# LabJunBMI/E3-invaraint-diffusion-model

Measured on AMD Instinct MI355X. Metric: denoising-steps/sec (batched pocket graphs), higher is better.
Workload: dtype f32 storage and accumulation, f16x3 products (fp32 grade); 1 GPU; structure_model sampling step, 256 x 256-residue pockets per GPU, 12+12 layers x 768, T=1000 schedule, encoder recomputed every step (as the reference); pockets_per_gpu=256, seq_len=256, parallelism=pocket-sharded x1, no collective

## Files before the change

e3-invaraint-diffusion-model_amd/csrc/attn_relkey_coop.hip:

```cpp
#include <type_traits>

#include "e3d_common.h"

namespace {

typedef __bf16 bf16x8 __attribute__((ext_vector_type(8)));
typedef __bf16 bf16x4 __attribute__((ext_vector_type(4)));
typedef _Float16 f16x8 __attribute__((ext_vector_type(8)));
typedef _Float16 f16x4 __attribute__((ext_vector_type(4)));
template <typename E> struct AV;
template <> struct AV<__bf16> { typedef bf16x8 x8; typedef bf16x4 x4; };
template <> struct AV<_Float16> { typedef f16x8 x8; typedef f16x4 x4; };
template <typename X> struct Elem;
template <> struct Elem<bf16x8> { typedef __bf16 type; };
template <> struct Elem<bf16x4> { typedef __bf16 type; };
template <> struct Elem<f16x8> { typedef _Float16 type; };
template <> struct Elem<f16x4> { typedef _Float16 type; };
__device__ __forceinline__ f32x16 mma16(const bf16x8 a, const bf16x8 b, const f32x16 c) {
    return __builtin_amdgcn_mfma_f32_32x32x16_bf16(a, b, c, 0, 0, 0);
}
__device__ __forceinline__ f32x16 mma16(const f16x8 a, const f16x8 b, const f32x16 c) {
    return __builtin_amdgcn_mfma_f32_32x32x16_f16(a, b, c, 0, 0, 0);
}

// ... 78 lines not shown
    const float* src = e + row * D + 16 * kb + 8 * (lane >> 5);
    typename AV<E>::x8 out;
    unsigned amax = 0;
#pragma unroll
    for (int t = 0; t < 8; ++t) {
        const float v = src[t];
        const E hi = (E)v;
        out[t] = plane ? (E)(v - (float)hi) : hi;
        e3d_absmax_accum(amax, v);
    }
    frag[i] = out;
    if (e_absmax && plane == 0) e3d_absmax_commit(amax, e_absmax, lane);
}

#ifdef E3D_ATTN_STAMPS
__device__ long long e3d_attn_stamps[16][8];
#define ASTAMP(slot)                                                                                     \
    do {                                                                                                 \
        if (blockIdx.x == 1000 && wid == 1 && lane == 0 && kt < 16) e3d_attn_stamps[kt][slot] = __builtin_readcyclecounter(); \
    } while (0)
#define KSTAMP(i)                                                                                        \
    do {                                                                                                 \
        if (blockIdx.x == 1000 && wid == 1 && lane == 0) e3d_attn_stamps[15][i] = __builtin_readcyclecounter(); \
    } while (0)
#else
#define ASTAMP(slot) do {} while (0)
#define KSTAMP(i) do {} while (0)
#endif

template <int W, bool RELKEY, typename E, bool DROP = false>
__global__ __launch_bounds__(W * 64, 2) void attn_coop_kernel(
    const float* __restrict__ q, int64_t q_bs, int64_t q_rs, const float* __restrict__ k, int64_t k_bs,
    int64_t k_rs, const float* __restrict__ v, int64_t v_bs, int64_t v_rs, const typename AV<E>::x8* __restrict__ e_frag,
    int P, const float* __restrict__ key_mask, float* __restrict__ out, float* __restrict__ lse, int nh, int Lq, int Lk,
    int groups_per_bh, int skip_padded_tiles, E3dBounds bnd, float rescale_tau, E3dDrop drop_in) {
    const E3dDrop drop = e3d_drop_resolve(drop_in);
    typedef typename AV<E>::x8 bf16x8;
    typedef typename AV<E>::x4 bf16x4;
    extern __shared__ __attribute__((aligned(16))) unsigned char smem_raw[];
    constexpr int NT = W * 64, NI = 512 / NT;
    const int tid = threadIdx.x, lane = tid & 63, wid = tid >> 6;
    const int qi = lane & 31, half = lane >> 5;
    const int blk = xcd_remap(blockIdx.x, gridDim.x);
    const int grp = blk % groups_per_bh, bh = blk / groups_per_bh, h = bh % nh, b = bh / nh;
    const int q0 = (grp * W + wid) * 32;
    float* ring = reinterpret_cast<float*>(smem_raw + 2 * KV_BUF_B) + wid * RING_F;
    KSTAMP(0);

    const float* kb_ = k + b * k_bs + h * D;
    const float* vb_ = v + b * v_bs + h * D;
    const float* mb = key_mask ? key_mask + (int64_t)b * Lk : nullptr;
    f32x4 qraw[8];
    {
        const float* qrow = q + b * q_bs + (int64_t)min(q0 + qi, Lq - 1) * q_rs + h * D + 8 * half;
#pragma unroll
        for (int kb = 0; kb < 4; ++kb) {
            qraw[2 * kb] = *reinterpret_cast<const f32x4*>(qrow + 16 * kb);
            qraw[2 * kb + 1] = *reinterpret_cast<const f32x4*>(qrow + 16 * kb + 4);
        }
    }
    uint64_t drop_row = 0;
    if (DROP) drop_row = e3d_drop_attn_row(drop, b, h, nh, Lq, Lk, min(q0 + qi, Lq - 1));
    const bool scan_mask = mb && skip_padded_tiles && e3d_mask_skip_is_exact(bnd);
    float mv[4];
    {
        const float* mp = mb ? mb : kb_;
#pragma unroll
        for (int c = 0; c < 4; ++c) mv[c] = mp[min(64 * c + lane, Lk - 1)];
    }

    bf16x8 qf[4][2];
    int k_tiles = (Lk + 31) >> 5;

    constexpr bool DEEP = NI <= 2;
    constexpr int NSET = DEEP ? 2 : 1;
    f32x4 sk[NSET][NI], sv[NSET][NI];
    float smask[NSET];
    int voff_k[NI], voff_v[NI];
#pragma unroll
    for (int i = 0; i < NI; ++i) {
        const int f = tid + NT * i;
        voff_k[i] = ((f >> 4) * (int)k_rs + 4 * (f & 15)) * 4;
        voff_v[i] = ((f >> 4) * (int)v_rs + 4 * (f & 15)) * 4;
    }
    const int voff_m = (tid & 31) * 4;
    auto tile_rsrc = [&](const float* base, int64_t rs, int r0, int tail_floats) {
        const int rows = Lk - r0;
        return __builtin_amdgcn_make_buffer_rsrc(const_cast<float*>(base + (int64_t)r0 * rs), 0,
                                                 (int)(((int64_t)(rows - 1) * rs + tail_floats) * 4), 0x00020000);
    };
    auto stage_load = [&](auto set_tag, int r0) {
        constexpr int SET = decltype(set_tag)::value;
        const auto rk = tile_rsrc(kb_, k_rs, r0, D), rv = tile_rsrc(vb_, v_rs, r0, D);
#pragma unroll
        for (int i = 0; i < NI; ++i) {
            sk[SET][i] = __builtin_bit_cast(f32x4, __builtin_amdgcn_raw_buffer_load_b128(rk, voff_k[i], 0, 0));
            sv[SET][i] = __builtin_bit_cast(f32x4, __builtin_amdgcn_raw_buffer_load_b128(rv, voff_v[i], 0, 0));
        }
        const auto rm = tile_rsrc(mb ? mb : kb_, 1, r0, 1);
        const float mval = __builtin_bit_cast(float, __builtin_amdgcn_raw_buffer_load_b32(rm, voff_m, 0, 0));
        smask[SET] = mb ? mval : 1.0f;
    };
    auto stage_store = [&](auto set_tag, int r0, unsigned char* buf) {
        constexpr int SET = decltype(set_tag)::value;
#pragma unroll
        for (int i = 0; i < NI; ++i) {
            const int f = tid + NT * i, row = f >> 4, c4 = f & 15;
            bf16x4 hi, lo;
            split4x2(sk[SET][i], hi, lo);
            *reinterpret_cast<bf16x4*>(buf + row * K_ROW_B + 8 * c4) = hi;
            *reinterpret_cast<bf16x4*>(buf + K_PLANE_B + row * K_ROW_B + 8 * c4) = lo;
            split4x2(sv[SET][i], hi, lo);
            *reinterpret_cast<bf16x4*>(buf + 2 * K_PLANE_B + row * V_ROW_B + 8 * c4) = hi;
            *reinterpret_cast<bf16x4*>(buf + 2 * K_PLANE_B + V_PLANE_B + row * V_ROW_B + 8 * c4) = lo;
        }
        if (tid < 32)
            reinterpret_cast<float*>(buf + 2 * K_PLANE_B + 2 * V_PLANE_B)[tid] =
                r0 + tid < Lk ? (1.0f - smask[SET]) * MASK_BIAS : -INFINITY;
    };
    using Set0 = std::integral_constant<int, 0>;
    using Set1 = std::integral_constant<int, DEEP ? 1 : 0>;

    bf16x8 ef[4][2];
    const int J0 = (Lk + 31) >> 5, qt = q0 >> 5;
    const auto e_rsrc = __builtin_amdgcn_make_buffer_rsrc(const_cast<bf16x8*>(e_frag ? e_frag : reinterpret_cast<const bf16x8*>(k)), 0,
                                                          2 * ((Lk + 31) >> 5) * 512 * 16, 0x00020000);
    const int voff_e = lane * 16;
    auto e_load = [&](int j) {
        const int so = __builtin_amdgcn_readfirstlane(j * 8192);
#pragma unroll
        for (int kb = 0; kb < 4; ++kb) {
            ef[kb][0] = __builtin_bit_cast(bf16x8, __builtin_amdgcn_raw_buffer_load_b128(e_rsrc, voff_e + kb * 1024, so, 0));
            ef[kb][1] = __builtin_bit_cast(bf16x8, __builtin_amdgcn_raw_buffer_load_b128(e_rsrc, voff_e + kb * 1024, so + 4096, 0));
        }
    };
    auto dot_q_acc = [&](const bf16x8 (&x)[4][2], f32x16 acc) {
#pragma unroll
        for (int kb = 0; kb < 4; ++kb) acc = mfma3(x[kb], qf[kb], acc);
        return acc;
    };
    auto dot_q = [&](const bf16x8 (&x)[4][2]) {
        f32x16 acc;
#pragma unroll
        for (int r = 0; r < 16; ++r) acc[r] = 0.f;
        return dot_q_acc(x, acc);
    };

    stage_load(Set0{}, 0);
    if (RELKEY) e_load(qt + J0);

    if (scan_mask) {
        int last = -1;
#pragma unroll
        for (int c = 0; c < 4; ++c) {
            const bool valid = 64 * c + lane < Lk && mv[c] != 0.f;
            const unsigned long long bits = __ballot(valid);
            if (bits) last = 64 * c + 63 - __builtin_clzll(bits);
        }
        for (int base = 256; base < Lk; base += 64) {
            const int key = base + lane;
            const bool valid = key < Lk && mb[key] != 0.f;
            const unsigned long long bits = __ballot(valid);
            if (bits) last = base + 63 - __builtin_clzll(bits);
        }
        if (last >= 0) k_tiles = (last >> 5) + 1;
    }
#pragma unroll
    for (int kb = 0; kb < 4; ++kb) {
        const f32x4 lo4 = qraw[2 * kb], hi4 = qraw[2 * kb + 1];
        float x[8] = {lo4[0] * Q_SCALE, lo4[1] * Q_SCALE, lo4[2] * Q_SCALE, lo4[3] * Q_SCALE,
                      hi4[0] * Q_SCALE, hi4[1] * Q_SCALE, hi4[2] * Q_SCALE, hi4[3] * Q_SCALE};
#pragma unroll
        for (int j = 0; j < 8; ++j) asm volatile("" : "+v"(x[j]));
        split8x2(x, qf[kb][0], qf[kb][1]);
    }
    if (RELKEY) {
        f32x16 t = dot_q(ef);
        e_load(qt - 1 + J0);
#pragma unroll
        for (int r = 0; r < 16; ++r) ring[(32 + mfma32_row(r, half)) * RING_LD + qi] = t[r];
        t = dot_q(ef);
        e_load(qt - (k_tiles > 1 ? 1 : 0) - 1 + J0);
#pragma unroll
        for (int r = 0; r < 16; ++r) ring[mfma32_row(r, half) * RING_LD + qi] = t[r];
    }
    stage_store(Set0{}, 0, smem_raw);
    if (DEEP) stage_load(Set1{}, (k_tiles > 1 ? 1 : 0) * 32);
    __syncthreads();
    KSTAMP(1);

    f32x16 o0, o1;
#pragma unroll
    for (int r = 0; r < 16; ++r) { o0[r] = 0.f; o1[r] = 0.f; }
    float m_run = 0.f, l_run = 0.f;
    float* const ring_w = ring + 4 * half * RING_LD + qi;
    const float* const ring_e = ring + (qi + 31 - 4 * half - 27) * RING_LD + qi;
    int rd_odd[16];
    if (RELKEY) {
#pragma unroll
        for (int r = 0; r < 16; ++r) rd_odd[r] = (((qi - mfma32_row(r, half) + 31) ^ 32) * RING_LD + qi);
    }

    auto tile = [&](auto par_tag, int kt) {
        constexpr int PAR = decltype(par_tag)::value;
        const unsigned char* buf = smem_raw + PAR * KV_BUF_B;
        const bool more = kt + 1 < k_tiles;
        const int kt_next = more ? kt + 1 : kt;
        ASTAMP(0);
        ASTAMP(1);

        const float* kbias = reinterpret_cast<const float*>(buf + 2 * K_PLANE_B + 2 * V_PLANE_B);
        f32x16 s;
#pragma unroll
        for (int g = 0; g < 4; ++g) {
            const f32x4 bv = *reinterpret_cast<const f32x4*>(kbias + 8 * g + 4 * half);
#pragma unroll
            for (int j = 0; j < 4; ++j) s[4 * g + j] = bv[j] - m_run;
        }
        if (RELKEY) {
#pragma unroll
            for (int r = 0; r < 16; ++r)
                s[r] += PAR ? ring[rd_odd[r]] : ring_e[(27 - ((r & 3) + 8 * (r >> 2))) * RING_LD];
        }
        {
            bf16x8 kf[4][2];
            const unsigned char* kr = buf + qi * K_ROW_B + 16 * half;
#pragma unroll
            for (int kb = 0; kb < 4; ++kb) {
                kf[kb][0] = *reinterpret_cast<const bf16x8*>(kr + 32 * kb);
                kf[kb][1] = *reinterpret_cast<const bf16x8*>(kr + K_PLANE_B + 32 * kb);
            }
            s = dot_q_acc(kf, s);
        }
        ASTAMP(2);
        const int kt_ld = DEEP ? (kt + 2 < k_tiles ? kt + 2 : k_tiles - 1) : kt_next;
        if (PAR == 0) stage_load(Set0{}, kt_ld * 32);
        else stage_load(Set1{}, kt_ld * 32);
        ASTAMP(3);

        float tmax = -INFINITY;
#pragma unroll
        for (int r = 0; r < 16; ++r) tmax = fmaxf(tmax, s[r]);
        tmax = fmaxf(tmax, __shfl_xor(tmax, 32, 64));
        const bool grow = kt == 0 || tmax > rescale_tau;
        if (__builtin_amdgcn_ballot_w64(grow) != 0ull) {
            const float delta = grow ? tmax : 0.f;
            const float alpha = kt == 0 ? 0.f : __builtin_amdgcn_exp2f(-delta);
            m_run += delta;
            l_run *= alpha;
#pragma unroll
            for (int r = 0; r < 16; ++r) { o0[r] *= alpha; o1[r] *= alpha; s[r] -= delta; }
        }
        float psum = 0.f;
#pragma unroll
        for (int r = 0; r < 16; ++r) {
            s[r] = __builtin_amdgcn_exp2f(s[r]);
            psum += s[r];
        }
        l_run += psum;
        if (DROP) {
#pragma unroll
            for (int g = 0; g < 4; ++g) {
                float m[4];
                e3d_drop_mult4_row(drop, drop_row, (uint32_t)(kt * 8 + 2 * g + half), m);
#pragma unroll
                for (int j = 0; j < 4; ++j) s[4 * g + j] *= m[j];
            }
        }
        ASTAMP(4);

        const unsigned char* vr = buf + 2 * K_PLANE_B + (4 * half + ((lane >> 2) & 3)) * V_ROW_B +
                                  2 * (16 * ((lane >> 4) & 1) + 4 * (lane & 3));
#pragma unroll
        for (int st = 0; st < 2; ++st) {
            float pv[8];
#pragma unroll
            for (int j = 0; j < 8; ++j) pv[j] = s[8 * st + j];
            bf16x8 pb[2], a0[2], a1[2];
            split8x2(pv, pb[0], pb[1]);
            const unsigned char* v0 = vr + 16 * st * V_ROW_B;
#pragma unroll
            for (int pl = 0; pl < 2; ++pl) {
                a0[pl] = tr_read8<bf16x8>(v0 + pl * V_PLANE_B, v0 + pl * V_PLANE_B + 8 * V_ROW_B);
                a1[pl] = tr_read8<bf16x8>(v0 + pl * V_PLANE_B + 64, v0 + pl * V_PLANE_B + 8 * V_ROW_B + 64);
            }
            o0 = mfma3(a0, pb, o0);
            o1 = mfma3(a1, pb, o1);
        }

        ASTAMP(5);
        if (more) {
            if (DEEP == (PAR == 0)) stage_store(Set1{}, kt_next * 32, smem_raw + (PAR ^ 1) * KV_BUF_B);
            else stage_store(Set0{}, kt_next * 32, smem_raw + (PAR ^ 1) * KV_BUF_B);
        }
        ASTAMP(6);
        if (RELKEY && more) {
            const f32x16 t = dot_q(ef);
            e_load(qt - (kt + 2 < k_tiles ? kt + 2 : k_tiles - 1) - 1 + J0);
#pragma unroll
            for (int r = 0; r < 16; ++r) ring_w[(32 * (PAR ^ 1) + (r & 3) + 8 * (r >> 2)) * RING_LD] = t[r];
        }
        __syncthreads();
        ASTAMP(7);
    };
    for (int kt = 0; kt < k_tiles; kt += 2) {
        tile(std::integral_constant<int, 0>{}, kt);
        if (kt + 1 < k_tiles) tile(std::integral_constant<int, 1>{}, kt + 1);
    }

    KSTAMP(2);
    const float l_tot = l_run + __shfl_xor(l_run, 32, 64);
    const float inv = 1.0f / l_tot;
    __builtin_amdgcn_wave_barrier();
#pragma unroll
    for (int g = 0; g < 4; ++g) {
        f32x4 a, c;
#pragma unroll
        for (int j = 0; j < 4; ++j) { a[j] = o0[4 * g + j] * inv; c[j] = o1[4 * g + j] * inv; }
        *reinterpret_cast<f32x4*>(ring + qi * OUT_LD + 8 * g + 4 * half) = a;
        *reinterpret_cast<f32x4*>(ring + qi * OUT_LD + 32 + 8 * g + 4 * half) = c;
    }
    __builtin_amdgcn_fence(__ATOMIC_RELEASE, "wavefront");
    __builtin_amdgcn_wave_barrier();
    __builtin_amdgcn_fence(__ATOMIC_ACQUIRE, "wavefront");
    float* obase = out + ((int64_t)b * Lq + q0) * (nh * D) + h * D;
#pragma unroll
    for (int i = 0; i < 8; ++i) {
        const int row = 4 * i + (lane >> 4);
        if (q0 + row < Lq)
            *reinterpret_cast<f32x4*>(obase + (int64_t)row * (nh * D) + 4 * (lane & 15)) =
                *reinterpret_cast<const f32x4*>(ring + row * OUT_LD + 4 * (lane & 15));
    }
    if (lse && half == 0 && q0 + qi < Lq) lse[((int64_t)b * nh + h) * Lq + q0 + qi] = m_run * LN2 + logf(l_tot);
    KSTAMP(3);
#ifdef E3D_ATTN_STAMPS
    asm volatile("s_waitcnt vmcnt(0)" ::: "memory");
    KSTAMP(4);
#endif
}

template <int W, bool RELKEY, typename E>
int launch_w(const float* q, int64_t q_bs, int64_t q_rs, const float* k, int64_t k_bs, int64_t k_rs, const float* v,
             int64_t v_bs, int64_t v_rs, const void* e_frag, int P, const float* key_mask,
             float* out, float* lse, int B, int nh, int Lq, int Lk, int q_tiles, int skip, E3dBounds bnd, E3dDrop drop,
             bool dropping, hipStream_t s) {
    const size_t lds = 2 * KV_BUF_B + (size_t)W * RING_F * sizeof(float);
    const int groups = q_tiles / W;
    if constexpr (std::is_same<E, __bf16>::value) {
        if (dropping) {
            static std::atomic<uint64_t> lds_ok_d{0};
            e3d_allow_lds(lds_ok_d, attn_coop_kernel<W, RELKEY, E, true>, lds);
            hipLaunchKernelGGL((attn_coop_kernel<W, RELKEY, E, true>), dim3(B * nh * groups), dim3(W * 64), lds, s, q, q_bs, q_rs,
                               k, k_bs, k_rs, v, v_bs, v_rs, reinterpret_cast<const typename AV<E>::x8*>(e_frag), P, key_mask,
                               out, lse, nh, Lq, Lk, groups, skip, bnd, g_rescale_tau, drop);
            return e3d_launch_status("e3d_relkey_attn_fwd_split (cooperative, dropout)");
        }
    }
    static std::atomic<uint64_t> lds_ok{0};
    e3d_allow_lds(lds_ok, attn_coop_kernel<W, RELKEY, E>, lds);
    hipLaunchKernelGGL((attn_coop_kernel<W, RELKEY, E>), dim3(B * nh * groups), dim3(W * 64), lds, s, q, q_bs, q_rs, k, k_bs,
                       k_rs, v, v_bs, v_rs, reinterpret_cast<const typename AV<E>::x8*>(e_frag), P, key_mask, out, lse, nh, Lq, Lk, groups, skip, bnd, g_rescale_tau, drop);
    return e3d_launch_status("e3d_relkey_attn_fwd_split (cooperative)");
}

template <bool RELKEY, typename E>
int launch_any(int W, const float* q, int64_t q_bs, int64_t q_rs, const float* k, int64_t k_bs, int64_t k_rs,
               const float* v, int64_t v_bs, int64_t v_rs, const void* e_frag, int P,
               const float* key_mask, float* out, float* lse, int B, int nh, int Lq, int Lk, int q_tiles, int skip,
               E3dBounds bnd, E3dDrop drop, bool dropping, hipStream_t s) {
#define E3D_COOP_CASE(w)                                                                                          \
    case w:                                                                                                       \
        return launch_w<w, RELKEY, E>(q, q_bs, q_rs, k, k_bs, k_rs, v, v_bs, v_rs, e_frag, P, key_mask, out, lse, B, nh, \
                                   Lq, Lk, q_tiles, skip, bnd, drop, dropping, s)
    switch (W) {
        E3D_COOP_CASE(8);
        E3D_COOP_CASE(4);
// ... 30 lines not shown
    return launch_any<true, E>(W, q, q_bs, q_rs, k, k_bs, k_rs, v, v_bs, v_rs, e_scratch, P, key_mask, out, lse, B, nh, Lq,
                               Lk, q_tiles, skip, bnd, drop, dropping, s);
}

int e3d_attn_coop_launch(const float* q, int64_t q_bs, int64_t q_rs, const float* k, int64_t k_bs, int64_t k_rs,
                         const float* v, int64_t v_bs, int64_t v_rs, const float* dist_emb, int P,
                         const float* key_mask, float* out, float* lse, int B, int nh, int Lq, int Lk, int skip,
                         E3dBounds bnd, void* e_scratch, int e_ready, int f16, E3dDrop drop, bool dropping, hipStream_t s) {
    if (f16)
        return coop_launch_t<_Float16>(q, q_bs, q_rs, k, k_bs, k_rs, v, v_bs, v_rs, dist_emb, P, key_mask, out, lse, B, nh, Lq,
                                       Lk, skip, bnd, e_scratch, e_ready, drop, dropping, s);
    return coop_launch_t<__bf16>(q, q_bs, q_rs, k, k_bs, k_rs, v, v_bs, v_rs, dist_emb, P, key_mask, out, lse, B, nh, Lq, Lk,
                                 skip, bnd, e_scratch, e_ready, drop, dropping, s);
}

extern "C" float e3d_attn_rescale_tau(float tau) {
    const float prev = g_rescale_tau;
    if (tau >= 0.f) g_rescale_tau = tau;
    return prev;
}

#ifdef E3D_ATTN_STAMPS
extern "C" int e3d_debug_read_attn_stamps(long long* host_out) {
    return (int)hipMemcpyFromSymbol(host_out, HIP_SYMBOL(e3d_attn_stamps), sizeof(long long) * 16 * 8);
}
#endif

int e3d_attn_fill_planes(const float* dist_emb, int P, int Lk, void* scratch, int f16, float* e_absmax, hipStream_t s) {
    const int J0 = (Lk + 31) / 32, n_items = 2 * J0 * 512;
    if (f16)
// ... 10 lines not shown
```

e3-invaraint-diffusion-model_amd/csrc/attn_relkey_split.hip:

```cpp
#include "attn_split_frag.h"

namespace {

template <int NS, bool RELKEY, bool DROP, typename E>
__global__ __launch_bounds__(256, 2) void attn_fwd_split_kernel(
    const float* __restrict__ q, int64_t q_bs, int64_t q_rs, const float* __restrict__ k, int64_t k_bs,
    int64_t k_rs, const float* __restrict__ v, int64_t v_bs, int64_t v_rs, const float* __restrict__ dist_emb,
    int P, const float* __restrict__ key_mask, float* __restrict__ out, float* __restrict__ lse, int nh, int Lq,
    int Lk, int q_tiles, int n_units, int skip_padded_tiles, E3dBounds bnd, E3dDrop drop_in) {
    const E3dDrop drop = e3d_drop_resolve(drop_in);
    typedef typename AV<E>::x8 bf16x8;
    extern __shared__ __attribute__((aligned(16))) float smem[];
    const int lane = threadIdx.x & 63, wid = threadIdx.x >> 6;
    const int qi = lane & 31, half = lane >> 5;
    const int unit = xcd_remap(blockIdx.x, gridDim.x) * (blockDim.x >> 6) + wid;
    if (unit >= n_units) return;
    const int qt = unit % q_tiles, bh = unit / q_tiles, h = bh % nh, b = bh / nh;
    float* ring = smem + wid * WAVE_LDS_F;
    float* stg = ring + RING_F;
    float* kbias = stg + STG_F;

    const int q0 = qt * 32;
    const int lq = min(q0 + qi, Lq - 1);
    uint64_t drop_row = 0;
// ... 190 lines not shown
    }
    E3D_REQUIRE((int64_t)B * nh * ((Lq + 31) / 32) < (1ll << 30), "attn_split: too many tiles");
    hipStream_t s = (hipStream_t)stream;
    if (dist_emb && e_scratch && !e_scratch_ready) {
        const int rc = e3d_attn_fill_planes(dist_emb, P, Lk, e_scratch, f16, e_absmax, s);
        if (rc) return rc;
        e_scratch_ready = 1;
    }
    static int coop = -1;
    if (coop < 0) {
        const char* e = getenv("E3D_ATTN_COOP");
        coop = e ? atoi(e) : 1;
    }
    const bool dropping = drop_p > 0.f;
    const bool span_ok = (int64_t)Lk * (k_rs > v_rs ? k_rs : v_rs) * 4 < ((int64_t)1 << 31) && k_rs > 0 && v_rs > 0 &&
                         k_rs < ((int64_t)1 << 24) && v_rs < ((int64_t)1 << 24);
    if ((terms == 3 || (f16 && !dropping)) && coop && span_ok && v_rs % 4 == 0 && v_bs % 4 == 0 && ((Lq + 31) / 32) % 4 == 0 &&
        (!dist_emb || e_scratch))
        return e3d_attn_coop_launch(q, q_bs, q_rs, k, k_bs, k_rs, v, v_bs, v_rs, dist_emb, P, key_mask, out, lse, B, nh,
                                    Lq, Lk, g_skip_padded, bnd, e_scratch, e_scratch_ready, f16, d, dropping, s);
    if (dropping) {
        if (terms == 3)
            return launch<2, true>(q, q_bs, q_rs, k, k_bs, k_rs, v, v_bs, v_rs, dist_emb, P, key_mask, out, lse, B, nh, Lq, Lk, bnd, s, d);
        return launch<3, true>(q, q_bs, q_rs, k, k_bs, k_rs, v, v_bs, v_rs, dist_emb, P, key_mask, out, lse, B, nh, Lq, Lk, bnd, s, d);
    }
    if (f16)
        return launch<2, false, _Float16>(q, q_bs, q_rs, k, k_bs, k_rs, v, v_bs, v_rs, dist_emb, P, key_mask, out, lse, B, nh,
                                          Lq, Lk, bnd, s);
    if (terms == 3)
        return launch<2>(q, q_bs, q_rs, k, k_bs, k_rs, v, v_bs, v_rs, dist_emb, P, key_mask, out, lse, B, nh, Lq, Lk, bnd, s);
    return launch<3>(q, q_bs, q_rs, k, k_bs, k_rs, v, v_bs, v_rs, dist_emb, P, key_mask, out, lse, B, nh, Lq, Lk, bnd, s);
// ... 53 lines not shown
```

e3-invaraint-diffusion-model_amd/hip.py:

```python
import ctypes
import os
from ctypes import c_char_p, c_float, c_int, c_int64, c_uint32, c_uint64, c_void_p

_HERE = os.path.dirname(os.path.abspath(__file__))
LIB_PATH = os.environ.get("E3D_HIP_LIB", os.path.join(_HERE, "libe3d_hip.so"))
ABI_VERSION = 5

_P = c_void_p
_SIGNATURES = {
    "e3d_abi_version": (c_int, []),
    "e3d_last_error": (c_char_p, []),
    "e3d_gemm_bias_act_f32": (c_int, [_P, c_int64, _P, _P, _P, c_int64, c_int, c_int, c_int, c_int, _P]),
    "e3d_gemm_bias_act_f32_split": (c_int, [_P, c_int64, _P, _P, _P, c_int64, c_int, c_int, c_int, c_int, c_int, _P]),
    "e3d_gemm_bias_act_f32_split_ex": (c_int, [_P, c_int64, _P, _P, _P, c_int64, c_int, c_int, c_int, c_int, c_int, _P, c_float, _P]),
    "e3d_absmax_f32": (c_int, [_P, c_int64, _P, _P]),
    "e3d_relkey_attn_fwd": (c_int, [_P, c_int64, c_int64, _P, c_int64, c_int64, _P, c_int64, c_int64,
                                    _P, c_int, _P, _P, _P, c_int, c_int, c_int, c_int, _P]),
    "e3d_relkey_attn_fwd_split": (c_int, [_P, c_int64, c_int64, _P, c_int64, c_int64, _P, c_int64, c_int64,
                                          _P, c_int, _P, _P, _P, c_int, c_int, c_int, c_int, c_int, _P]),
    "e3d_gemm_skinny_workspace_bytes": (c_int64, [c_int, c_int, c_int]),
    "e3d_gemm_skinny_f32_split": (c_int, [_P, c_int64, _P, _P, _P, c_int64, c_int, c_int, c_int, c_int, c_int, _P, c_int64, _P]),
    "e3d_gemm_skinny_f32_split_ex": (c_int, [_P, c_int64, _P, _P, _P, c_int64, c_int, c_int, c_int, c_int, c_int, _P, c_int64, _P, c_float, _P]),
    "e3d_gemm_skinny_plan_select": (None, [c_int, c_int]),
    "e3d_gemm_skinny_residual_layernorm_f32_split": (c_int, [_P, c_int64, _P, _P, _P, _P, _P, c_float, _P, c_int, c_int, c_int,
                                                     c_int, _P, c_int64, _P]),
    "e3d_gemm_skinny_residual_layernorm_f32_split_ex": (c_int, [_P, c_int64, _P, _P, _P, _P, _P, c_float, _P, c_int, c_int, c_int,
                                                        c_int, _P, c_int64, c_float, _P]),
    "e3d_attn_skip_padded_tiles": (c_int, [c_int]),
    "e3d_gemm_kernel_select": (c_int, [c_int]),
    "e3d_gemm_general_select": (c_int, [c_int]),
    "e3d_attn_rescale_tau": (c_float, [c_float]),
    "e3d_residual_layernorm_fwd": (c_int, [_P, _P, _P, _P, c_float, _P, _P, c_int, c_int, _P]),
    "e3d_adaln_gate_fwd": (c_int, [_P, _P, _P, c_int, c_int, _P, c_int, c_int, _P]),
    "e3d_embed_layernorm_fwd": (c_int, [_P, c_int, _P, _P, _P, _P, c_float, _P, c_int, _P, _P, c_int, c_int, _P]),
    "e3d_nerf_backbone": (c_int, [_P, _P, _P, c_int, c_int, c_int, _P]),
    "e3d_gemm_f32_split_general": (c_int, [_P, c_int64, c_int, _P, c_int64, c_int, _P, _P, c_int64, c_int, c_int,
                                           c_int, c_int, c_int, _P]),
    "e3d_transpose_grouped_f32": (c_int, [_P, _P, c_int, c_int, c_int, c_int64, c_int64, _P]),
    "e3d_gemm_wgrad_grouped_f32_split": (c_int, [_P, _P, _P, _P, c_uint64, c_int, c_int64, c_int64, c_int, c_int, c_int, c_int, _P]),
    "e3d_residual_layernorm_drop_fwd": (c_int, [_P, _P, _P, _P, c_float, _P, _P, c_int, c_int, c_float, c_uint64, _P]),
    "e3d_layernorm_bwd_drop": (c_int, [_P, _P, _P, c_float, _P, _P, _P, _P, c_int, c_int, c_float, c_uint64, _P]),
    "e3d_weight_planes_bytes": (c_int64, [c_int, c_int]),
    "e3d_weight_planes_f32_split": (c_int, [_P, c_int, c_int, c_int, _P, _P]),
# ... 106 lines not shown
```

include/e3d_hip.h:

```cpp
#ifndef E3D_HIP_H
#define E3D_HIP_H

#include <stdint.h>

#ifdef __cplusplus
extern "C" {
#endif

#define E3D_ABI_VERSION 5

#define E3D_TERMS_BF16 1
#define E3D_TERMS_BF16X3 3
#define E3D_TERMS_BF16X6 6
#define E3D_TERMS_F16X3 19

#define E3D_ACT_NONE 0
#define E3D_ACT_GELU 1
#define E3D_ACT_SILU 2

int e3d_abi_version(void);
const char* e3d_last_error(void);

int e3d_gemm_bias_act_f32(const float* A, int64_t lda, const float* W, const float* bias,
                          float* out, int64_t ldc, int M, int N, int K, int act, void* stream);
// ... 32 lines not shown
                                                 const float* residual, const float* gamma, const float* beta, float eps,
                                                 float* out, int M, int H, int K, int terms, void* workspace,
                                                 int64_t workspace_bytes, void* stream);
int e3d_gemm_skinny_residual_layernorm_f32_split_ex(const float* A, int64_t lda, const float* W, const float* bias,
                                                    const float* residual, const float* gamma, const float* beta,
                                                    float eps, float* out, int M, int H, int K, int terms,
                                                    void* workspace, int64_t workspace_bytes, float out_scale,
                                                    void* stream);

int e3d_gemm_kernel_select(int pref);
int e3d_gemm_general_select(int form);

float e3d_attn_rescale_tau(float tau);

int e3d_attn_skip_padded_tiles(int enable);

int e3d_residual_layernorm_fwd(const float* x, const float* residual, const float* gamma,
                               const float* beta, float eps, float* s_out, float* out, int M,
                               int H, void* stream);

int e3d_adaln_gate_fwd(const float* x, const float* y, const float* mod, int branch,
                       int rows_per_cond, float* out, int M, int H, void* stream);

int e3d_embed_layernorm_fwd(const float* x, int F, const float* W, const float* b,
                            const float* gamma, const float* beta, float eps,
                            const float* post_add, int rows_per_add, float* z_out, float* out,
                            int M, int H, void* stream);

int e3d_head_linear_fwd(const float* x, const float* W, const float* b, float* out, int M,
                        int H, int Nout, void* stream);
// ... 203 lines not shown
```

Baseline: 3982 pocket-steps/s.

## Make cooperative relkey attention kernel persistent with cross-item K/V prefetch

```diff
diff --git a/e3-invaraint-diffusion-model_amd/csrc/attn_relkey_coop.hip b/e3-invaraint-diffusion-model_amd/csrc/attn_relkey_coop.hip
--- a/e3-invaraint-diffusion-model_amd/csrc/attn_relkey_coop.hip
+++ b/e3-invaraint-diffusion-model_amd/csrc/attn_relkey_coop.hip
@@ -116,18 +116,23 @@
 }
 
 #ifdef E3D_ATTN_STAMPS
+#ifndef E3D_ATTN_STAMP_ITEM
+#define E3D_ATTN_STAMP_ITEM 1000
+#endif
 __device__ long long e3d_attn_stamps[16][8];
 #define ASTAMP(slot)                                                                                     \
     do {                                                                                                 \
-        if (blockIdx.x == 1000 && wid == 1 && lane == 0 && kt < 16) e3d_attn_stamps[kt][slot] = __builtin_readcyclecounter(); \
+        if (item == E3D_ATTN_STAMP_ITEM && wid == 1 && lane == 0 && kt < 16) e3d_attn_stamps[kt][slot] = __builtin_readcyclecounter(); \
     } while (0)
-#define KSTAMP(i)                                                                                        \
+#define KSTAMP_AT(id, i)                                                                                 \
     do {                                                                                                 \
-        if (blockIdx.x == 1000 && wid == 1 && lane == 0) e3d_attn_stamps[15][i] = __builtin_readcyclecounter(); \
+        if ((id) == E3D_ATTN_STAMP_ITEM && wid == 1 && lane == 0) e3d_attn_stamps[15][i] = __builtin_readcyclecounter(); \
     } while (0)
+#define KSTAMP(i) KSTAMP_AT(item, i)
 #else
 #define ASTAMP(slot) do {} while (0)
 #define KSTAMP(i) do {} while (0)
+#define KSTAMP_AT(id, i) do {} while (0)
 #endif
 
 template <int W, bool RELKEY, typename E, bool DROP = false>
@@ -135,7 +140,7 @@
     const float* __restrict__ q, int64_t q_bs, int64_t q_rs, const float* __restrict__ k, int64_t k_bs,
     int64_t k_rs, const float* __restrict__ v, int64_t v_bs, int64_t v_rs, const typename AV<E>::x8* __restrict__ e_frag,
     int P, const float* __restrict__ key_mask, float* __restrict__ out, float* __restrict__ lse, int nh, int Lq, int Lk,
-    int groups_per_bh, int skip_padded_tiles, E3dBounds bnd, float rescale_tau, E3dDrop drop_in) {
+    int groups_per_bh, int n_items, int skip_padded_tiles, E3dBounds bnd, float rescale_tau, E3dDrop drop_in) {
     const E3dDrop drop = e3d_drop_resolve(drop_in);
     typedef typename AV<E>::x8 bf16x8;
     typedef typename AV<E>::x4 bf16x4;
@@ -143,41 +148,31 @@
     constexpr int NT = W * 64, NI = 512 / NT;
     const int tid = threadIdx.x, lane = tid & 63, wid = tid >> 6;
     const int qi = lane & 31, half = lane >> 5;
-    const int blk = xcd_remap(blockIdx.x, gridDim.x);
-    const int grp = blk % groups_per_bh, bh = blk / groups_per_bh, h = bh % nh, b = bh / nh;
-    const int q0 = (grp * W + wid) * 32;
     float* ring = reinterpret_cast<float*>(smem_raw + 2 * KV_BUF_B) + wid * RING_F;
-    KSTAMP(0);
-
-    const float* kb_ = k + b * k_bs + h * D;
-    const float* vb_ = v + b * v_bs + h * D;
-    const float* mb = key_mask ? key_mask + (int64_t)b * Lk : nullptr;
+
+    struct Item { int b, h, q0; const float* kp; const float* vp; const float* mp; };
+    auto decode = [&](int id) {
+        const int blk = xcd_remap(id, n_items);
+        const int grp = blk % groups_per_bh, bh = blk / groups_per_bh;
+        Item t;
+        t.h = bh % nh;
+        t.b = bh / nh;
+        t.q0 = (grp * W + wid) * 32;
+        t.kp = k + t.b * k_bs + t.h * D;
+        t.vp = v + t.b * v_bs + t.h * D;
+        t.mp = key_mask ? key_mask + (int64_t)t.b * Lk : nullptr;
+        return t;
+    };
+    const bool scan_mask = key_mask && skip_padded_tiles && e3d_mask_skip_is_exact(bnd);
+
     f32x4 qraw[8];
-    {
-        const float* qrow = q + b * q_bs + (int64_t)min(q0 + qi, Lq - 1) * q_rs + h * D + 8 * half;
-#pragma unroll
-        for (int kb = 0; kb < 4; ++kb) {
-            qraw[2 * kb] = *reinterpret_cast<const f32x4*>(qrow + 16 * kb);
-            qraw[2 * kb + 1] = *reinterpret_cast<const f32x4*>(qrow + 16 * kb + 4);
-        }
-    }
+    bf16x8 qf[4][2];
     uint64_t drop_row = 0;
-    if (DROP) drop_row = e3d_drop_attn_row(drop, b, h, nh, Lq, Lk, min(q0 + qi, Lq - 1));
-    const bool scan_mask = mb && skip_padded_tiles && e3d_mask_skip_is_exact(bnd);
     float mv[4];
-    {
-        const float* mp = mb ? mb : kb_;
-#pragma unroll
-        for (int c = 0; c < 4; ++c) mv[c] = mp[min(64 * c + lane, Lk - 1)];
-    }
-
-    bf16x8 qf[4][2];
-    int k_tiles = (Lk + 31) >> 5;
-
-    constexpr bool DEEP = NI <= 2;
-    constexpr int NSET = DEEP ? 2 : 1;
-    f32x4 sk[NSET][NI], sv[NSET][NI];
-    float smask[NSET];
+
+    static_assert(NI <= 2, "two staging register sets: 4 or 8 waves per workgroup");
+    f32x4 sk[2][NI], sv[2][NI];
+    float smask[2];
     int voff_k[NI], voff_v[NI];
 #pragma unroll
     for (int i = 0; i < NI; ++i) {
@@ -191,17 +186,17 @@
         return __builtin_amdgcn_make_buffer_rsrc(const_cast<float*>(base + (int64_t)r0 * rs), 0,
                                                  (int)(((int64_t)(rows - 1) * rs + tail_floats) * 4), 0x00020000);
     };
-    auto stage_load = [&](auto set_tag, int r0) {
+    auto stage_load = [&](auto set_tag, const float* kp, const float* vp, const float* mp, int r0) {
         constexpr int SET = decltype(set_tag)::value;
-        const auto rk = tile_rsrc(kb_, k_rs, r0, D), rv = tile_rsrc(vb_, v_rs, r0, D);
+        const auto rk = tile_rsrc(kp, k_rs, r0, D), rv = tile_rsrc(vp, v_rs, r0, D);
 #pragma unroll
         for (int i = 0; i < NI; ++i) {
             sk[SET][i] = __builtin_bit_cast(f32x4, __builtin_amdgcn_raw_buffer_load_b128(rk, voff_k[i], 0, 0));
             sv[SET][i] = __builtin_bit_cast(f32x4, __builtin_amdgcn_raw_buffer_load_b128(rv, voff_v[i], 0, 0));
         }
-        const auto rm = tile_rsrc(mb ? mb : kb_, 1, r0, 1);
+        const auto rm = tile_rsrc(mp ? mp : kp, 1, r0, 1);
         const float mval = __builtin_bit_cast(float, __builtin_amdgcn_raw_buffer_load_b32(rm, voff_m, 0, 0));
-        smask[SET] = mb ? mval : 1.0f;
+        smask[SET] = mval;
     };
     auto stage_store = [&](auto set_tag, int r0, unsigned char* buf) {
         constexpr int SET = decltype(set_tag)::value;
@@ -218,13 +213,13 @@
         }
         if (tid < 32)
             reinterpret_cast<float*>(buf + 2 * K_PLANE_B + 2 * V_PLANE_B)[tid] =
-                r0 + tid < Lk ? (1.0f - smask[SET]) * MASK_BIAS : -INFINITY;
+                tid < Lk - r0 ? (1.0f - (key_mask ? smask[SET] : 1.0f)) * MASK_BIAS : -INFINITY;
     };
     using Set0 = std::integral_constant<int, 0>;
-    using Set1 = std::integral_constant<int, DEEP ? 1 : 0>;
+    using Set1 = std::integral_constant<int, 1>;
 
     bf16x8 ef[4][2];
-    const int J0 = (Lk + 31) >> 5, qt = q0 >> 5;
+    const int J0 = (Lk + 31) >> 5;
     const auto e_rsrc = __builtin_amdgcn_make_buffer_rsrc(const_cast<bf16x8*>(e_frag ? e_frag : reinterpret_cast<const bf16x8*>(k)), 0,
                                                           2 * ((Lk + 31) >> 5) * 512 * 16, 0x00020000);
     const int voff_e = lane * 16;
@@ -248,53 +243,6 @@
         return dot_q_acc(x, acc);
     };
 
-    stage_load(Set0{}, 0);
-    if (RELKEY) e_load(qt + J0);
-
-    if (scan_mask) {
-        int last = -1;
-#pragma unroll
-        for (int c = 0; c < 4; ++c) {
-            const bool valid = 64 * c + lane < Lk && mv[c] != 0.f;
-            const unsigned long long bits = __ballot(valid);
-            if (bits) last = 64 * c + 63 - __builtin_clzll(bits);
-        }
-        for (int base = 256; base < Lk; base += 64) {
-            const int key = base + lane;
-            const bool valid = key < Lk && mb[key] != 0.f;
-            const unsigned long long bits = __ballot(valid);
-            if (bits) last = base + 63 - __builtin_clzll(bits);
-        }
-        if (last >= 0) k_tiles = (last >> 5) + 1;
-    }
-#pragma unroll
-    for (int kb = 0; kb < 4; ++kb) {
-        const f32x4 lo4 = qraw[2 * kb], hi4 = qraw[2 * kb + 1];
-        float x[8] = {lo4[0] * Q_SCALE, lo4[1] * Q_SCALE, lo4[2] * Q_SCALE, lo4[3] * Q_SCALE,
-                      hi4[0] * Q_SCALE, hi4[1] * Q_SCALE, hi4[2] * Q_SCALE, hi4[3] * Q_SCALE};
-#pragma unroll
-        for (int j = 0; j < 8; ++j) asm volatile("" : "+v"(x[j]));
-        split8x2(x, qf[kb][0], qf[kb][1]);
-    }
-    if (RELKEY) {
-        f32x16 t = dot_q(ef);
-        e_load(qt - 1 + J0);
-#pragma unroll
-        for (int r = 0; r < 16; ++r) ring[(32 + mfma32_row(r, half)) * RING_LD + qi] = t[r];
-        t = dot_q(ef);
-        e_load(qt - (k_tiles > 1 ? 1 : 0) - 1 + J0);
-#pragma unroll
-        for (int r = 0; r < 16; ++r) ring[mfma32_row(r, half) * RING_LD + qi] = t[r];
-    }
-    stage_store(Set0{}, 0, smem_raw);
-    if (DEEP) stage_load(Set1{}, (k_tiles > 1 ? 1 : 0) * 32);
-    __syncthreads();
-    KSTAMP(1);
-
-    f32x16 o0, o1;
-#pragma unroll
-    for (int r = 0; r < 16; ++r) { o0[r] = 0.f; o1[r] = 0.f; }
-    float m_run = 0.f, l_run = 0.f;
     float* const ring_w = ring + 4 * half * RING_LD + qi;
     const float* const ring_e = ring + (qi + 31 - 4 * half - 27) * RING_LD + qi;
     int rd_odd[16];
@@ -303,142 +251,271 @@
         for (int r = 0; r < 16; ++r) rd_odd[r] = (((qi - mfma32_row(r, half) + 31) ^ 32) * RING_LD + qi);
     }
 
-    auto tile = [&](auto par_tag, int kt) {
-        constexpr int PAR = decltype(par_tag)::value;
-        const unsigned char* buf = smem_raw + PAR * KV_BUF_B;
-        const bool more = kt + 1 < k_tiles;
-        const int kt_next = more ? kt + 1 : kt;
-        ASTAMP(0);
-        ASTAMP(1);
-
-        const float* kbias = reinterpret_cast<const float*>(buf + 2 * K_PLANE_B + 2 * V_PLANE_B);
-        f32x16 s;
+    auto item_loads = [&](const Item& t) {
+        int ln = lane;
+        asm volatile("" : "+v"(ln));
+        const float* mp = t.mp ? t.mp : t.kp;
+#pragma unroll
+        for (int c = 0; c < 4; ++c) mv[c] = mp[min(64 * c + ln, Lk - 1)];
+        const int row = min(t.q0 + (ln & 31), Lq - 1);
+        const float* qrow = q + t.b * q_bs + (int64_t)row * q_rs + t.h * D + 8 * (ln >> 5);
+#pragma unroll
+        for (int kb = 0; kb < 4; ++kb) {
+            qraw[2 * kb] = *reinterpret_cast<const f32x4*>(qrow + 16 * kb);
+            qraw[2 * kb + 1] = *reinterpret_cast<const f32x4*>(qrow + 16 * kb + 4);
+        }
+        if (DROP) drop_row = e3d_drop_attn_row(drop, t.b, t.h, nh, Lq, Lk, row);
+        if (RELKEY) e_load((t.q0 >> 5) + J0);
+    };
+
+    auto item_prologue = [&](const Item& it, int item, bool have_t1) {
+        int k_tiles = J0;
+        const int qt = it.q0 >> 5;
+        if (scan_mask) {
+            int last = -1;
+#pragma unroll
+            for (int c = 0; c < 4; ++c) {
+                const bool valid = 64 * c + lane < Lk && mv[c] != 0.f;
+                const unsigned long long bits = __ballot(valid);
+                if (bits) last = 64 * c + 63 - __builtin_clzll(bits);
+            }
+            int ln = lane;
+            asm volatile("" : "+v"(ln));
+            for (int base = 256; base < Lk; base += 64) {
+                const int key = base + ln;
+                const bool valid = key < Lk && it.mp[key] != 0.f;
+                const unsigned long long bits = __ballot(valid);
+                if (bits) last = base + 63 - __builtin_clzll(bits);
+            }
+            if (last >= 0) k_tiles = (last >> 5) + 1;
+        }
+#pragma unroll
+        for (int kb = 0; kb < 4; ++kb) {
+            const f32x4 lo4 = qraw[2 * kb], hi4 = qraw[2 * kb + 1];
+            float x[8] = {lo4[0] * Q_SCALE, lo4[1] * Q_SCALE, lo4[2] * Q_SCALE, lo4[3] * Q_SCALE,
+                          hi4[0] * Q_SCALE, hi4[1] * Q_SCALE, hi4[2] * Q_SCALE, hi4[3] * Q_SCALE};
+#pragma unroll
+            for (int j = 0; j < 8; ++j) asm volatile("" : "+v"(x[j]));
+            split8x2(x, qf[kb][0], qf[kb][1]);
+        }
+#pragma unroll
+        for (int c = 0; c < 4; ++c) asm volatile("" ::"v"(mv[c]));
+        if (RELKEY) {
+            f32x16 t = dot_q(ef);
+            e_load(qt - 1 + J0);
+#pragma unroll
+            for (int r = 0; r < 16; ++r) ring_w[(32 + (r & 3) + 8 * (r >> 2)) * RING_LD] = t[r];
+            t = dot_q(ef);
+            e_load(qt - (k_tiles > 1 ? 1 : 0) - 1 + J0);
+#pragma unroll
+            for (int r = 0; r < 16; ++r) ring_w[((r & 3) + 8 * (r >> 2)) * RING_LD] = t[r];
+        }
+        stage_store(Set0{}, 0, smem_raw);
+        if (!have_t1) stage_load(Set1{}, it.kp, it.vp, it.mp, (k_tiles > 1 ? 1 : 0) * 32);
+        __syncthreads();
+        KSTAMP(1);
+        return k_tiles;
+    };
+
+    int item = blockIdx.x;
+    Item cur = decode(item);
+    KSTAMP(0);
+    stage_load(Set0{}, cur.kp, cur.vp, cur.mp, 0);
+    item_loads(cur);
+    int k_tiles = item_prologue(cur, item, false);
+
+    for (;;) {
+        const int item_next = item + (int)gridDim.x;
+        const bool has_next = item_next < n_items;
+        const Item nxt = decode(has_next ? item_next : item);
+        const int q0 = cur.q0, qt = q0 >> 5;
+        const float* const kb_ = cur.kp;
+        const float* const vb_ = cur.vp;
+        const float* const mb = cur.mp;
+
+        f32x16 o0, o1;
+#pragma unroll
+        for (int r = 0; r < 16; ++r) { o0[r] = 0.f; o1[r] = 0.f; }
+        float m_run = 0.f, l_run = 0.f;
+
+        auto tile = [&](auto par_tag, int kt) {
+            constexpr int PAR = decltype(par_tag)::value;
+            const unsigned char* buf = smem_raw + PAR * KV_BUF_B;
+            const bool more = kt + 1 < k_tiles;
+            const int kt_next = more ? kt + 1 : kt;
+            ASTAMP(0);
+            ASTAMP(1);
+
+            const float* kbias = reinterpret_cast<const float*>(buf + 2 * K_PLANE_B + 2 * V_PLANE_B);
+            f32x16 s;
+#pragma unroll
+            for (int g = 0; g < 4; ++g) {
+                const f32x4 bv = *reinterpret_cast<const f32x4*>(kbias + 8 * g + 4 * half);
+#pragma unroll
+                for (int j = 0; j < 4; ++j) s[4 * g + j] = bv[j] - m_run;
+            }
+            if (RELKEY) {
+#pragma unroll
+                for (int r = 0; r < 16; ++r)
+                    s[r] += PAR ? ring[rd_odd[r]] : ring_e[(27 - ((r & 3) + 8 * (r >> 2))) * RING_LD];
+            }
+            {
+                bf16x8 kf[4][2];
+                const unsigned char* kr = buf + qi * K_ROW_B + 16 * half;
+#pragma unroll
+                for (int kb = 0; kb < 4; ++kb) {
+                    kf[kb][0] = *reinterpret_cast<const bf16x8*>(kr + 32 * kb);
+                    kf[kb][1] = *reinterpret_cast<const bf16x8*>(kr + K_PLANE_B + 32 * kb);
+                }
+                s = dot_q_acc(kf, s);
+            }
+            ASTAMP(2);
+            {
+                const bool in_item = kt + 2 < k_tiles;
+                const bool to_next = !in_item && has_next;
+                const int kt_ld = in_item ? kt + 2 : (to_next ? (PAR < J0 ? PAR : J0 - 1) : k_tiles - 1);
+                if (PAR == 0) stage_load(Set0{}, to_next ? nxt.kp : kb_, to_next ? nxt.vp : vb_, to_next ? nxt.mp : mb, kt_ld * 32);
+                else stage_load(Set1{}, to_next ? nxt.kp : kb_, to_next ? nxt.vp : vb_, to_next ? nxt.mp : mb, kt_ld * 32);
+            }
+            ASTAMP(3);
+
+            float tmax = -INFINITY;
+#pragma unroll
+            for (int r = 0; r < 16; ++r) tmax = fmaxf(tmax, s[r]);
+            tmax = fmaxf(tmax, __shfl_xor(tmax, 32, 64));
+            const bool grow = kt == 0 || tmax > rescale_tau;
+            if (__builtin_amdgcn_ballot_w64(grow) != 0ull) {
+                const float delta = grow ? tmax : 0.f;
+                const float alpha = kt == 0 ? 0.f : __builtin_amdgcn_exp2f(-delta);
+                m_run += delta;
+                l_run *= alpha;
+#pragma unroll
+                for (int r = 0; r < 16; ++r) { o0[r] *= alpha; o1[r] *= alpha; s[r] -= delta; }
+            }
+            float psum = 0.f;
+#pragma unroll
+            for (int r = 0; r < 16; ++r) {
+                s[r] = __builtin_amdgcn_exp2f(s[r]);
+                psum += s[r];
+            }
+            l_run += psum;
+            if (DROP) {
+#pragma unroll
+                for (int g = 0; g < 4; ++g) {
+                    float m[4];
+                    e3d_drop_mult4_row(drop, drop_row, (uint32_t)(kt * 8 + 2 * g + half), m);
+#pragma unroll
+                    for (int j = 0; j < 4; ++j) s[4 * g + j] *= m[j];
+                }
+            }
+            ASTAMP(4);
+
+            const unsigned char* vr = buf + 2 * K_PLANE_B + (4 * half + ((lane >> 2) & 3)) * V_ROW_B +
+                                      2 * (16 * ((lane >> 4) & 1) + 4 * (lane & 3));
+#pragma unroll
+            for (int st = 0; st < 2; ++st) {
+                float pv[8];
+#pragma unroll
+                for (int j = 0; j < 8; ++j) pv[j] = s[8 * st + j];
+                bf16x8 pb[2], a0[2], a1[2];
+                split8x2(pv, pb[0], pb[1]);
+                const unsigned char* v0 = vr + 16 * st * V_ROW_B;
+#pragma unroll
+                for (int pl = 0; pl < 2; ++pl) {
+                    a0[pl] = tr_read8<bf16x8>(v0 + pl * V_PLANE_B, v0 + pl * V_PLANE_B + 8 * V_ROW_B);
+                    a1[pl] = tr_read8<bf16x8>(v0 + pl * V_PLANE_B + 64, v0 + pl * V_PLANE_B + 8 * V_ROW_B + 64);
+                }
+                o0 = mfma3(a0, pb, o0);
+                o1 = mfma3(a1, pb, o1);
+            }
+
+            ASTAMP(5);
+            if (more) {
+                if (PAR == 0) stage_store(Set1{}, kt_next * 32, smem_raw + (PAR ^ 1) * KV_BUF_B);
+                else stage_store(Set0{}, kt_next * 32, smem_raw + (PAR ^ 1) * KV_BUF_B);
+            }
+            ASTAMP(6);
+            if (RELKEY && more) {
+                const f32x16 t = dot_q(ef);
+                e_load(qt - (kt + 2 < k_tiles ? kt + 2 : k_tiles - 1) - 1 + J0);
+#pragma unroll
+                for (int r = 0; r < 16; ++r) ring_w[(32 * (PAR ^ 1) + (r & 3) + 8 * (r >> 2)) * RING_LD] = t[r];
+            }
+            __syncthreads();
+            ASTAMP(7);
+        };
+        for (int kt = 0; kt < k_tiles; kt += 2) {
+            tile(std::integral_constant<int, 0>{}, kt);
+            if (kt + 1 < k_tiles) tile(std::integral_constant<int, 1>{}, kt + 1);
+        }
+
+        KSTAMP(2);
+        const bool have_t1 = has_next && k_tiles >= 2;
+        const int b_out = cur.b, h_out = cur.h;
+        item_loads(nxt);
+
+        const float l_tot = l_run + __shfl_xor(l_run, 32, 64);
+        const float inv = 1.0f / l_tot;
+        int ln = lane;
+        asm volatile("" : "+v"(ln));
+        float* otile = ring + (ln & 31) * OUT_LD + 4 * (ln >> 5);
+        __builtin_amdgcn_wave_barrier();
 #pragma unroll
         for (int g = 0; g < 4; ++g) {
-            const f32x4 bv = *reinterpret_cast<const f32x4*>(kbias + 8 * g + 4 * half);
-#pragma unroll
-            for (int j = 0; j < 4; ++j) s[4 * g + j] = bv[j] - m_run;
-        }
-        if (RELKEY) {
-#pragma unroll
-            for (int r = 0; r < 16; ++r)
-                s[r] += PAR ? ring[rd_odd[r]] : ring_e[(27 - ((r & 3) + 8 * (r >> 2))) * RING_LD];
-        }
+            f32x4 a, c;
+#pragma unroll
+            for (int j = 0; j < 4; ++j) { a[j] = o0[4 * g + j] * inv; c[j] = o1[4 * g + j] * inv; }
+            *reinterpret_cast<f32x4*>(otile + 8 * g) = a;
+            *reinterpret_cast<f32x4*>(otile + 32 + 8 * g) = c;
+        }
+        __builtin_amdgcn_fence(__ATOMIC_RELEASE, "wavefront");
+        __builtin_amdgcn_wave_barrier();
+        __builtin_amdgcn_fence(__ATOMIC_ACQUIRE, "wavefront");
+        const int row0 = ln >> 4;
+        const auto o_rsrc = __builtin_amdgcn_make_buffer_rsrc(out + (int64_t)b_out * Lq * (nh * D) + h_out * D, 0,
+                                                              (int)((((int64_t)Lq - 1) * (nh * D) + D) * 4), 0x00020000);
+        const int voff_o = ((q0 + row0) * (nh * D) + 4 * (ln & 15)) * 4;
+        const float* rrow = ring + row0 * OUT_LD + 4 * (ln & 15);
+        typedef decltype(__builtin_amdgcn_raw_buffer_load_b128(o_rsrc, 0, 0, 0)) raw128;
+#pragma unroll
+        for (int i = 0; i < 8; ++i)
+            __builtin_amdgcn_raw_buffer_store_b128(__builtin_bit_cast(raw128, *reinterpret_cast<const f32x4*>(rrow + 4 * i * OUT_LD)),
+                                                   o_rsrc, voff_o + 4 * i * (nh * D) * 4, 0, 0);
         {
-            bf16x8 kf[4][2];
-            const unsigned char* kr = buf + qi * K_ROW_B + 16 * half;
-#pragma unroll
-            for (int kb = 0; kb < 4; ++kb) {
-                kf[kb][0] = *reinterpret_cast<const bf16x8*>(kr + 32 * kb);
-                kf[kb][1] = *reinterpret_cast<const bf16x8*>(kr + K_PLANE_B + 32 * kb);
-            }
-            s = dot_q_acc(kf, s);
-        }
-        ASTAMP(2);
-        const int kt_ld = DEEP ? (kt + 2 < k_tiles ? kt + 2 : k_tiles - 1) : kt_next;
-        if (PAR == 0) stage_load(Set0{}, kt_ld * 32);
-        else stage_load(Set1{}, kt_ld * 32);
-        ASTAMP(3);
-
-        float tmax = -INFINITY;
-#pragma unroll
-        for (int r = 0; r < 16; ++r) tmax = fmaxf(tmax, s[r]);
-        tmax = fmaxf(tmax, __shfl_xor(tmax, 32, 64));
-        const bool grow = kt == 0 || tmax > rescale_tau;
-        if (__builtin_amdgcn_ballot_w64(grow) != 0ull) {
-            const float delta = grow ? tmax : 0.f;
-            const float alpha = kt == 0 ? 0.f : __builtin_amdgcn_exp2f(-delta);
-            m_run += delta;
-            l_run *= alpha;
-#pragma unroll
-            for (int r = 0; r < 16; ++r) { o0[r] *= alpha; o1[r] *= alpha; s[r] -= delta; }
-        }
-        float psum = 0.f;
-#pragma unroll
-        for (int r = 0; r < 16; ++r) {
-            s[r] = __builtin_amdgcn_exp2f(s[r]);
-            psum += s[r];
-        }
-        l_run += psum;
-        if (DROP) {
-#pragma unroll
-            for (int g = 0; g < 4; ++g) {
-                float m[4];
-                e3d_drop_mult4_row(drop, drop_row, (uint32_t)(kt * 8 + 2 * g + half), m);
-#pragma unroll
-                for (int j = 0; j < 4; ++j) s[4 * g + j] *= m[j];
-            }
-        }
-        ASTAMP(4);
-
-        const unsigned char* vr = buf + 2 * K_PLANE_B + (4 * half + ((lane >> 2) & 3)) * V_ROW_B +
-                                  2 * (16 * ((lane >> 4) & 1) + 4 * (lane & 3));
-#pragma unroll
-        for (int st = 0; st < 2; ++st) {
-            float pv[8];
-#pragma unroll
-            for (int j = 0; j < 8; ++j) pv[j] = s[8 * st + j];
-            bf16x8 pb[2], a0[2], a1[2];
-            split8x2(pv, pb[0], pb[1]);
-            const unsigned char* v0 = vr + 16 * st * V_ROW_B;
-#pragma unroll
-            for (int pl = 0; pl < 2; ++pl) {
-                a0[pl] = tr_read8<bf16x8>(v0 + pl * V_PLANE_B, v0 + pl * V_PLANE_B + 8 * V_ROW_B);
-                a1[pl] = tr_read8<bf16x8>(v0 + pl * V_PLANE_B + 64, v0 + pl * V_PLANE_B + 8 * V_ROW_B + 64);
-            }
-            o0 = mfma3(a0, pb, o0);
-            o1 = mfma3(a1, pb, o1);
-        }
-
-        ASTAMP(5);
-        if (more) {
-            if (DEEP == (PAR == 0)) stage_store(Set1{}, kt_next * 32, smem_raw + (PAR ^ 1) * KV_BUF_B);
-            else stage_store(Set0{}, kt_next * 32, smem_raw + (PAR ^ 1) * KV_BUF_B);
-        }
-        ASTAMP(6);
-        if (RELKEY && more) {
-            const f32x16 t = dot_q(ef);
-            e_load(qt - (kt + 2 < k_tiles ? kt + 2 : k_tiles - 1) - 1 + J0);
-#pragma unroll
-            for (int r = 0; r < 16; ++r) ring_w[(32 * (PAR ^ 1) + (r & 3) + 8 * (r >> 2)) * RING_LD] = t[r];
-        }
-        __syncthreads();
-        ASTAMP(7);
-    };
-    for (int kt = 0; kt < k_tiles; kt += 2) {
-        tile(std::integral_constant<int, 0>{}, kt);
-        if (kt + 1 < k_tiles) tile(std::integral_constant<int, 1>{}, kt + 1);
-    }
-
-    KSTAMP(2);
-    const float l_tot = l_run + __shfl_xor(l_run, 32, 64);
-    const float inv = 1.0f / l_tot;
-    __builtin_amdgcn_wave_barrier();
-#pragma unroll
-    for (int g = 0; g < 4; ++g) {
-        f32x4 a, c;
-#pragma unroll
-        for (int j = 0; j < 4; ++j) { a[j] = o0[4 * g + j] * inv; c[j] = o1[4 * g + j] * inv; }
-        *reinterpret_cast<f32x4*>(ring + qi * OUT_LD + 8 * g + 4 * half) = a;
-        *reinterpret_cast<f32x4*>(ring + qi * OUT_LD + 32 + 8 * g + 4 * half) = c;
-    }
-    __builtin_amdgcn_fence(__ATOMIC_RELEASE, "wavefront");
-    __builtin_amdgcn_wave_barrier();
-    __builtin_amdgcn_fence(__ATOMIC_ACQUIRE, "wavefront");
-    float* obase = out + ((int64_t)b * Lq + q0) * (nh * D) + h * D;
-#pragma unroll
-    for (int i = 0; i < 8; ++i) {
-        const int row = 4 * i + (lane >> 4);
-        if (q0 + row < Lq)
-            *reinterpret_cast<f32x4*>(obase + (int64_t)row * (nh * D) + 4 * (lane & 15)) =
-                *reinterpret_cast<const f32x4*>(ring + row * OUT_LD + 4 * (lane & 15));
-    }
-    if (lse && half == 0 && q0 + qi < Lq) lse[((int64_t)b * nh + h) * Lq + q0 + qi] = m_run * LN2 + logf(l_tot);
-    KSTAMP(3);
+            const auto l_rsrc = __builtin_amdgcn_make_buffer_rsrc(lse ? lse + ((int64_t)b_out * nh + h_out) * Lq : out, 0,
+                                                                  lse ? Lq * 4 : 0, 0x00020000);
+            const float lval = m_run * LN2 + logf(l_tot);
+            __builtin_amdgcn_raw_buffer_store_b32(__builtin_bit_cast(decltype(__builtin_amdgcn_raw_buffer_load_b32(l_rsrc, 0, 0, 0)), lval),
+                                                  l_rsrc, ln < 32 ? (q0 + ln) * 4 : 0x7ffffff0, 0, 0);
+        }
+        KSTAMP(3);
+        if (!has_next) break;
+        __builtin_amdgcn_fence(__ATOMIC_RELEASE, "wavefront");
+        __builtin_amdgcn_wave_barrier();
+        KSTAMP(4);
+        item = item_next;
+        cur = nxt;
+        KSTAMP(0);
+        k_tiles = item_prologue(cur, item, have_t1);
+    }
 #ifdef E3D_ATTN_STAMPS
     asm volatile("s_waitcnt vmcnt(0)" ::: "memory");
     KSTAMP(4);
 #endif
+}
+
+int g_attn_persistent = -1;
+int g_attn_persistent_grid = 0;
+
+int coop_grid(int items, size_t lds) {
+    if (g_attn_persistent < 0) {
+        const char* e = getenv("E3D_ATTN_PERSIST");
+        g_attn_persistent = e ? (atoi(e) != 0) : 1;
+    }
+    if (!g_attn_persistent) return items;
+    const int resident = g_attn_persistent_grid > 0 ? g_attn_persistent_grid
+                                                    : e3d_cu_count() * (2 * lds <= (size_t)160 * 1024 ? 2 : 1);
+    return items < resident ? items : resident;
 }
 
 template <int W, bool RELKEY, typename E>
@@ -447,21 +524,23 @@
              float* out, float* lse, int B, int nh, int Lq, int Lk, int q_tiles, int skip, E3dBounds bnd, E3dDrop drop,
              bool dropping, hipStream_t s) {
     const size_t lds = 2 * KV_BUF_B + (size_t)W * RING_F * sizeof(float);
-    const int groups = q_tiles / W;
+    const int groups = q_tiles / W, items = B * nh * groups;
+    const int grid = coop_grid(items, lds);
     if constexpr (std::is_same<E, __bf16>::value) {
         if (dropping) {
             static std::atomic<uint64_t> lds_ok_d{0};
             e3d_allow_lds(lds_ok_d, attn_coop_kernel<W, RELKEY, E, true>, lds);
-            hipLaunchKernelGGL((attn_coop_kernel<W, RELKEY, E, true>), dim3(B * nh * groups), dim3(W * 64), lds, s, q, q_bs, q_rs,
+            hipLaunchKernelGGL((attn_coop_kernel<W, RELKEY, E, true>), dim3(grid), dim3(W * 64), lds, s, q, q_bs, q_rs,
                                k, k_bs, k_rs, v, v_bs, v_rs, reinterpret_cast<const typename AV<E>::x8*>(e_frag), P, key_mask,
-                               out, lse, nh, Lq, Lk, groups, skip, bnd, g_rescale_tau, drop);
+                               out, lse, nh, Lq, Lk, groups, items, skip, bnd, g_rescale_tau, drop);
             return e3d_launch_status("e3d_relkey_attn_fwd_split (cooperative, dropout)");
         }
     }
     static std::atomic<uint64_t> lds_ok{0};
     e3d_allow_lds(lds_ok, attn_coop_kernel<W, RELKEY, E>, lds);
-    hipLaunchKernelGGL((attn_coop_kernel<W, RELKEY, E>), dim3(B * nh * groups), dim3(W * 64), lds, s, q, q_bs, q_rs, k, k_bs,
-                       k_rs, v, v_bs, v_rs, reinterpret_cast<const typename AV<E>::x8*>(e_frag), P, key_mask, out, lse, nh, Lq, Lk, groups, skip, bnd, g_rescale_tau, drop);
+    hipLaunchKernelGGL((attn_coop_kernel<W, RELKEY, E>), dim3(grid), dim3(W * 64), lds, s, q, q_bs, q_rs, k, k_bs,
+                       k_rs, v, v_bs, v_rs, reinterpret_cast<const typename AV<E>::x8*>(e_frag), P, key_mask, out, lse, nh, Lq, Lk,
+                       groups, items, skip, bnd, g_rescale_tau, drop);
     return e3d_launch_status("e3d_relkey_attn_fwd_split (cooperative)");
 }
 
@@ -522,6 +601,18 @@
                                  skip, bnd, e_scratch, e_ready, drop, dropping, s);
 }
 
+extern "C" int e3d_attn_persistent(int mode) {
+    (void)coop_grid(1, 0);
+    const int prev = g_attn_persistent;
+    if (mode >= 0) g_attn_persistent = mode != 0;
+    return prev;
+}
+extern "C" int e3d_attn_persistent_grid(int n) {
+    const int prev = g_attn_persistent_grid;
+    if (n >= 0) g_attn_persistent_grid = n;
+    return prev;
+}
+
 extern "C" float e3d_attn_rescale_tau(float tau) {
     const float prev = g_rescale_tau;
     if (tau >= 0.f) g_rescale_tau = tau;
diff --git a/e3-invaraint-diffusion-model_amd/csrc/attn_relkey_split.hip b/e3-invaraint-diffusion-model_amd/csrc/attn_relkey_split.hip
--- a/e3-invaraint-diffusion-model_amd/csrc/attn_relkey_split.hip
+++ b/e3-invaraint-diffusion-model_amd/csrc/attn_relkey_split.hip
@@ -228,7 +228,8 @@
     }
     const bool dropping = drop_p > 0.f;
     const bool span_ok = (int64_t)Lk * (k_rs > v_rs ? k_rs : v_rs) * 4 < ((int64_t)1 << 31) && k_rs > 0 && v_rs > 0 &&
-                         k_rs < ((int64_t)1 << 24) && v_rs < ((int64_t)1 << 24);
+                         k_rs < ((int64_t)1 << 24) && v_rs < ((int64_t)1 << 24) &&
+                         (int64_t)(Lq + 128) * nh * 64 * 4 < ((int64_t)1 << 31);
     if ((terms == 3 || (f16 && !dropping)) && coop && span_ok && v_rs % 4 == 0 && v_bs % 4 == 0 && ((Lq + 31) / 32) % 4 == 0 &&
         (!dist_emb || e_scratch))
         return e3d_attn_coop_launch(q, q_bs, q_rs, k, k_bs, k_rs, v, v_bs, v_rs, dist_emb, P, key_mask, out, lse, B, nh,
diff --git a/e3-invaraint-diffusion-model_amd/hip.py b/e3-invaraint-diffusion-model_amd/hip.py
--- a/e3-invaraint-diffusion-model_amd/hip.py
+++ b/e3-invaraint-diffusion-model_amd/hip.py
@@ -27,6 +27,8 @@
     "e3d_gemm_skinny_residual_layernorm_f32_split_ex": (c_int, [_P, c_int64, _P, _P, _P, _P, _P, c_float, _P, c_int, c_int, c_int,
                                                         c_int, _P, c_int64, c_float, _P]),
     "e3d_attn_skip_padded_tiles": (c_int, [c_int]),
+    "e3d_attn_persistent": (c_int, [c_int]),
+    "e3d_attn_persistent_grid": (c_int, [c_int]),
     "e3d_gemm_kernel_select": (c_int, [c_int]),
     "e3d_gemm_general_select": (c_int, [c_int]),
     "e3d_attn_rescale_tau": (c_float, [c_float]),
diff --git a/include/e3d_hip.h b/include/e3d_hip.h
--- a/include/e3d_hip.h
+++ b/include/e3d_hip.h
@@ -70,6 +70,10 @@
 float e3d_attn_rescale_tau(float tau);
 
 int e3d_attn_skip_padded_tiles(int enable);
+
+int e3d_attn_persistent(int mode);
+
+int e3d_attn_persistent_grid(int n);
 
 int e3d_residual_layernorm_fwd(const float* x, const float* residual, const float* gamma,
                                const float* beta, float eps, float* s_out, float* out, int M,
```

Result: no change. 3980 pocket-steps/s (-0.0%).
